# marksgraham/ddpm-ood

Hardware: AMD Instinct MI355X
Metric: reconstructions/sec (whole node), FashionMNIST 32x32 (higher is better)
Workload: dtype f32 (split-f16 MFMA products, fp32 accumulate)

## Files before the change

### ddpm_ood_amd/csrc/conv_wino44r.hip

```cpp
#include "wino44h_common.h"

namespace ddpm {

namespace {

constexpr int kVCB = 3 * kVSB;
static_assert(2 * kVCB == kRINGF * 4, "the V ring is the epilogue's four exchange slabs");

typedef int v4i_t __attribute__((ext_vector_type(4)));
typedef float v2f_t __attribute__((ext_vector_type(2)));

template <int O>
__device__ __forceinline__ void v_store_row_addtid(int m0base, const uint32_t (&hi6)[6], const uint32_t (&lo6)[6]) {
  asm volatile("s_mov_b32 m0, %0\n\ts_nop 1" ::"s"(m0base));
#pragma unroll
  for (int q = 0; q < 6; ++q) {
    asm volatile("ds_write_addtid_b32 %0 offset:%1" ::"v"(hi6[q]), "n"((2 * (O + q)) * (kT * 16)) : "memory");
    asm volatile("ds_write_addtid_b32 %0 offset:%1" ::"v"(lo6[q]), "n"((2 * (O + q) + 1) * (kT * 16)) : "memory");
  }
}

template <class T>
__device__ __forceinline__ const T *uniform_ptr(const T *p) {
  const uint64_t v = reinterpret_cast<uint64_t>(p);
  const uint32_t lo = __builtin_amdgcn_readfirstlane((uint32_t)v), hi = __builtin_amdgcn_readfirstlane((uint32_t)(v >> 32));
  return reinterpret_cast<const T *>(((uint64_t)hi << 32) | lo);
}

}

template <bool AFFINE, int NRT, int UIT, bool RES, bool D3 = false, bool UP = false>
__global__ __launch_bounds__(512, 2) void conv_wino44r_kernel(const ddpm_conv_desc a, const W44HGeom g) {
  extern __shared__ __attribute__((aligned(16))) float smem[];
  constexpr bool ONEIMG = UIT == 0;
  constexpr int NGS = ONEIMG ? 1 : NRT / UIT;
  constexpr int GD = ONEIMG ? NRT : UIT;
  float *const P = smem + kRINGF;

  const int tid = threadIdx.x;
  const int lane = tid & 63, wave = __builtin_amdgcn_readfirstlane(tid >> 6);
  const int l31 = lane & 31, lhi = lane >> 5;
  const int cb = wave & 1, pg = wave >> 1;
  const bool lateprod = wave < 4;
  const bool silu = a.act == DDPM_ACT_SILU;

  const int xcd = blockIdx.x & 7, wj = blockIdx.x >> 3;
  int kt = wj % g.KT, slot = (wj / g.KT) * 8 + xcd;
  if (g.xmap) {
    kt = xcd % g.KT;
    slot = wj * (8 / g.KT) + xcd / g.KT;
  }
  if (slot >= g.NS) return;
  const int split = slot % g.S;
  slot /= g.S;
  const int part = slot % g.parts, it0 = (slot / g.parts) * g.IPW;
  const int nitems = min(g.IPW, g.NIT - it0);
  const int r0 = part * g.TR;
  const int n_first = it0 * g.TI, n_end = n_first + nitems * g.TI;
  const int istep = g.rev ? -g.TI : g.TI;
  const int NCHs = g.NCH / g.S, ch_lo = split * NCHs;
  float *const outp = a.out + (size_t)split * g.pstride;

  f32x16 acc8;
  reserve_agprs();

  const __amdgpu_buffer_rsrc_t rs_u = __builtin_amdgcn_make_buffer_rsrc(
      const_cast<uint16_t *>(a.w_wino44h), 0, (int)((size_t)kX * a.Cout * g.Cin * g.nkd_w * 4), 0x00020000);
  const int ukt = ((kt * g.nkd_w + g.kd0) * g.NCHc + ch_lo) * 3;
  int ua = (3 * pg * 2 + lhi) * (kK * 16) + (cb * 32 + l31) * 16;
  int va = 3 * pg * (2 * kT * 16) + l31 * 16;

  auto barrier = [&]() __attribute__((always_inline)) {
    asm volatile("s_waitcnt lgkmcnt(0)\n\ts_barrier" ::: "memory");
    __builtin_amdgcn_sched_barrier(0);
  };
  auto zero_accumulators = [&]() __attribute__((always_inline)) {
    zero_pinned_tiles();
    float z;
    asm volatile("v_mov_b32 %0, 0" : "=v"(z));
    acc8 = f32x16{z, z, z, z, z, z, z, z, z, z, z, z, z, z, z, z};
  };

#ifdef W44R_PROBE
  if (blockIdx.x == 0 && lane == 0 && a.scratch) reinterpret_cast<unsigned long long *>(a.scratch)[512 + wave * 32 + 31] = __builtin_readcyclecounter();
#endif
  auto zero_borders = [&]() __attribute__((always_inline)) {
    const v4f z4 = {0.f, 0.f, 0.f, 0.f};
    for (int i = tid; i < g.HS; i += 512) *reinterpret_cast<v4f *>(P + 4 * i) = z4;
    __syncthreads();
  };

  using I0 = std::integral_constant<int, 0>;
  using I1 = std::integral_constant<int, 1>;
  using I2 = std::integral_constant<int, 2>;

#ifdef W44R_PROBE
  int probe_cc = -100;
  int n_idx_probe = 0;
#define W44R_STAMP(i)                                                                                                  \
  if (blockIdx.x == 0 && probe_cc >= 4 && probe_cc < 8 && lane == 0 && a.scratch)                                      \
    reinterpret_cast<unsigned long long *>(a.scratch)[((wave * 4 + (probe_cc - 4)) * 16 + (i)) & 511] = __builtin_readcyclecounter();
#define W44R_FSTAMP(i)                                                                                                 \
  if (blockIdx.x == 0 && n_idx_probe == 0 && lane == 0 && a.scratch)                                                    \
    reinterpret_cast<unsigned long long *>(a.scratch)[512 + wave * 32 + (i)] = __builtin_readcyclecounter();
#else
#define W44R_STAMP(i)
#define W44R_FSTAMP(i)
#endif
  W44R_FSTAMP(0)
  const int ptask = (wave & 3) == 3 ? -1 : wave - (wave >> 2);
  const int pst = (ptask & 1) * 16 + (lane >> 2), pj = lane & 3;
  int tb0;
  {
    const int per = g.TR * g.TWc;
    const int ti = pst / per, rem = pst - ti * per;
    const int tr = rem / g.TWc, tc = rem - tr * g.TWc;
    tb0 = (pj >> 1) * g.HS + 2 * (pj & 1) * g.PCH + ti * g.IS + 4 * tr * g.PW + 4 * tc;
  }
  int vw0 = pst * 16 + 4 * pj;
  auto produce = [&](auto tc_, int cc) __attribute__((always_inline)) {
    constexpr int t = decltype(tc_)::value;
    constexpr bool t0 = t == 0;
    constexpr float c1 = t0 ? -5.f : t == 1 ? -2.f : -0.5f, c2 = t0 ? 4.f : c1, bm = t0 ? 0.f : t == 1 ? 1.f : 2.f;
    asm volatile("" : "+v"(tb0), "+v"(vw0));
    const int pb0 = tb0 + (cc & 1) * 2 * g.HS;
    float cA[2][6], cB[2][6];
#pragma unroll
    for (int c = 0; c < 2; ++c) {
      const float *p = P + pb0 + c * g.PCH;
      float d4[6], d2[6], dx[6], dy[6], dz[6], dw[6];
      auto row = [&](int r, float (&dst)[6]) __attribute__((always_inline)) {
        const v4f lo = *reinterpret_cast<const v4f *>(p + r * g.PW);
        const v2f_t hi = *reinterpret_cast<const v2f_t *>(p + r * g.PW + 4);
        dst[0] = lo[0]; dst[1] = lo[1]; dst[2] = lo[2]; dst[3] = lo[3]; dst[4] = hi[0]; dst[5] = hi[1];
      };
      row(4, d4);
      row(2, d2);
      row(1, dw);
      row(t0 ? 5 : 3, dy);
      if (t0) {
        row(0, dx);
        row(3, dz);
      } else {
#pragma unroll
        for (int q = 0; q < 6; ++q) dx[q] = d2[q], dz[q] = dw[q];
      }
#pragma unroll
      for (int q = 0; q < 6; ++q) {
        const float wa = __builtin_fmaf(c2, dx[q], __builtin_fmaf(c1, d2[q], d4[q]));
        const float qq = __builtin_fmaf(c2, dw[q], __builtin_fmaf(c1, dz[q], dy[q]));
        cA[c][q] = __builtin_fmaf(bm, qq, wa);
        cB[c][q] = t0 ? qq : __builtin_fmaf(-bm, qq, wa);
      }
    }
    int vwa = vw0 + (cc & 1) * kVCB + t * kVSB;
    asm volatile("" : "+v"(vwa));
    float t0r[6], t1r[6];
    uint32_t hi6[6], lo6[6];
    bt6(cA[0], t0r);
    bt6(cA[1], t1r);
#pragma unroll
    for (int q = 0; q < 6; ++q) split_pair(t0r[q], t1r[q], hi6[q], lo6[q]);
    const int m0base = __builtin_amdgcn_readfirstlane((cc & 1) * kVCB + t * kVSB + (ptask & 1) * 256);
    v_store_row_addtid<0>(m0base, hi6, lo6);
    bt6(cB[0], t0r);
    bt6(cB[1], t1r);
#pragma unroll
    for (int q = 0; q < 6; ++q) split_pair(t0r[q], t1r[q], hi6[q], lo6[q]);
    v_store_row_addtid<6>(m0base, hi6, lo6);
  };
  auto produce_task = [&](int cc) __attribute__((always_inline)) {
    if (ptask < 0) return;
    const int t = ptask >> 1;
    if (t == 0) produce(I0{}, cc);
    else if (t == 1) produce(I1{}, cc);
    else produce(I2{}, cc);
  };

  const int sc = wave & 3, phalf = wave >> 2;
  const int row_lo = max(0, 4 * r0 - 1), row_hi = min(a.Ho, 4 * (r0 + g.TR) + 1);
  const int npx = (row_hi - row_lo) * a.Wo;
  const int dump = 4 * g.PCH + 1 + lane;
  int pix0, pw0, pixL = 0, pwL = 0;
  {
    const int e0 = lane;
    const bool valid = e0 < npx;
    auto src_of = [&](int row, int col) __attribute__((always_inline)) { return UP ? ((row >> 1) * (a.Wo >> 1) + (col >> 1)) * 4 : (row * a.Wo + col) * 4; };
    pix0 = valid ? src_of(row_lo + e0 / a.Wo, e0 % a.Wo) : (int)0x80000000;
    pw0 = valid ? sc * g.PCH + (row_lo + e0 / a.Wo - (4 * r0 - 1)) * g.PW + e0 % a.Wo + 1 : dump;
    if (ONEIMG) {
      const int eL = e0 + 64 * (NRT - 1);
      const bool vL = eL < npx;
      pixL = vL ? src_of(row_lo + eL / a.Wo, eL % a.Wo) : (int)0x80000000;
      pwL = vL ? sc * g.PCH + (row_lo + eL / a.Wo - (4 * r0 - 1)) * g.PW + eL % a.Wo + 1 : dump;
    }
  }
  const int prs = (64 / a.Wo) * g.PW;
  constexpr int kRoundBytes = UP ? 64 : 256;
  auto pix_of = [&](int k) __attribute__((always_inline)) { return ONEIMG ? (k == NRT - 1 ? pixL : pix0 + kRoundBytes * k) : pix0 + kRoundBytes * (k % GD); };
  auto pw_of = [&](int k) __attribute__((always_inline)) { return ONEIMG ? (k == NRT - 1 ? pwL : pw0 + k * prs) : pw0 + (k % GD) * prs + (k / GD) * g.IS; };
  const int bytes1 = a.B * a.C1 * (D3 ? g.CS : UP ? g.HWin : g.HW) * 4, bytes2 = a.B * a.C2 * g.HW * 4;
  const __amdgpu_buffer_rsrc_t rs_sc =
      __builtin_amdgcn_make_buffer_rsrc(const_cast<float *>(a.gscale), 0, AFFINE ? a.B * g.Cin * 4 : 0, 0x00020000);
  const __amdgpu_buffer_rsrc_t rs_sh =
      __builtin_amdgcn_make_buffer_rsrc(const_cast<float *>(a.gshift), 0, AFFINE ? a.B * g.Cin * 4 : 0, 0x00020000);
  int vzero;
  asm volatile("v_mov_b32 %0, 0" : "=v"(vzero));
  constexpr bool PACKED = UIT == 1;
  constexpr int NGL = PACKED ? 1 : NGS;
  float praw[2][NRT];
  float gs[2][NGL], gh[2][NGL];
  struct LoadCtx {
    __amdgpu_buffer_rsrc_t rs;
    int n_it, cx, cgl, cga, soff3;
    bool dok;
  };
  auto load_prep = [&](int cc, int n_cur, bool has_next) __attribute__((always_inline)) {
    LoadCtx L;
    const bool nxt = cc >= NCHs && has_next;
    const int cl = nxt ? cc - NCHs : min(max(cc, 0), NCHs - 1);
    L.n_it = nxt ? n_cur + istep : n_cur;
    int cg = (ch_lo + cl) * kC + phalf * 4 + sc;
    L.cga = cg;
    L.soff3 = 0;
    L.dok = true;
    if (D3) {
      const int kdi = cl / g.NCHc;
      cg = (cl - kdi * g.NCHc) * kC + phalf * 4 + sc;
      const int ni = min(L.n_it, g.NIMG - 1);
      const int nb = ni / g.D, dsl = ni - nb * g.D + g.kd0 + kdi - 1;
      L.dok = dsl >= 0 && dsl < g.D;
      L.soff3 = ((nb * a.C1 + cg) * g.D + (L.dok ? dsl : 0)) * g.HW * 4;
    }
    const bool first = cg < a.C1;
    L.rs = __builtin_amdgcn_make_buffer_rsrc(const_cast<float *>(first ? a.in1 : a.in2), 0, first ? bytes1 : bytes2, 0x00020000);
    L.cx = first ? a.C1 : a.C2;
    L.cgl = first ? cg : cg - a.C1;
    return L;
  };
  auto load_round = [&](const LoadCtx &L, auto setc, int k) __attribute__((always_inline)) {
    constexpr int S = decltype(setc)::value;
    const int ni = min(L.n_it + (ONEIMG ? 0 : k / GD), g.NIMG - 1);
    const int soff = D3 ? L.soff3 : (ni * L.cx + L.cgl) * (UP ? g.HWin : g.HW) * 4;
    const int voff = D3 && !L.dok ? (int)0x80000000 : pix_of(k);
    praw[S][k] = __builtin_bit_cast(float, __builtin_amdgcn_raw_buffer_load_b32(L.rs, voff, soff, 0));
  };
  auto load_affine = [&](const LoadCtx &L, auto setc, int i) __attribute__((always_inline)) {
    constexpr int S = decltype(setc)::value;
    if (AFFINE) {
      const int nb = min(L.n_it + i, g.NIMG - 1);
      const int goff = (nb * g.Cin + L.cga) * 4;
      const int voff = PACKED ? max(0, min(lane & 7, g.NIMG - 1 - L.n_it)) * (g.Cin * 4) : vzero;
      gs[S][i] = __builtin_bit_cast(float, __builtin_amdgcn_raw_buffer_load_b32(rs_sc, voff, goff, 0));
      gh[S][i] = __builtin_bit_cast(float, __builtin_amdgcn_raw_buffer_load_b32(rs_sh, voff, goff, 0));
    }
  };
  auto load_stage = [&](auto setc, int cc, int n_cur, bool has_next) __attribute__((always_inline)) {
    const LoadCtx L = load_prep(cc, n_cur, has_next);
#pragma unroll
    for (int k = 0; k < NRT; ++k) load_round(L, setc, k);
#pragma unroll
    for (int i = 0; i < NGL; ++i) load_affine(L, setc, i);
  };
  auto activate_round = [&](auto setc, int cc, int k) __attribute__((always_inline)) {
    constexpr int S = decltype(setc)::value;
    float *const Pr = P + (2 * (cc & 1) + phalf) * g.HS + pw_of(k);
    float sa = 0.f, sb = 0.f, ta = 0.f, tb = 0.f;
    if (AFFINE) {
      if (PACKED) {
        sa = __builtin_bit_cast(float, __builtin_amdgcn_readlane(__builtin_bit_cast(int, gs[S][0]), k / GD));
        sb = __builtin_bit_cast(float, __builtin_amdgcn_readlane(__builtin_bit_cast(int, gh[S][0]), k / GD));
      } else {
        sa = gs[S][k / GD];
        sb = gh[S][k / GD];
      }
      ta = -1.44269504088896341f * sa;
      tb = -1.44269504088896341f * sb;
    }
    auto act = [&](float x) __attribute__((always_inline)) {
      if (AFFINE) {
        const float v = __builtin_fmaf(x, sa, sb);
        const float t = __builtin_fmaf(x, ta, tb);
        return (kVScale * v) * __builtin_amdgcn_rcpf(1.0f + __builtin_amdgcn_exp2f(t));
      }
      return kVScaleRaw * (silu ? silu_fast(x) : x);
    };
    Pr[0] = act(praw[S][k]);
  };
  auto activate_stage = [&](auto setc, int cc) __attribute__((always_inline)) {
    asm volatile("" : "+v"(pix0), "+v"(pw0), "+v"(pixL), "+v"(pwL));
#pragma unroll
    for (int k = 0; k < NRT; ++k) activate_round(setc, cc, k);
  };

  constexpr int kAR = 6;
  h8 Ar[kAR];
  auto load_a = [&](int cl, int jj) __attribute__((always_inline)) {
    const int t = jj / 3, i = jj - 3 * t;
    const int c2 = min(cl, NCHs - 1);
    const v4i_t v = __builtin_bit_cast(v4i_t, __builtin_amdgcn_raw_buffer_load_b128(rs_u, ua + i * (2 * kK * 16), (ukt + 3 * c2 + t) * kUSB, 0));
    return __builtin_bit_cast(h8, v);
  };
  auto mfma_chunk = [&](auto parc, int cl, auto &&slice) __attribute__((always_inline)) {
    constexpr int PAR = decltype(parc)::value;
    asm volatile("" : "+v"(ua), "+v"(va));
    const int vb = va + (cl & 1) * kVCB;
    h8 Bh[2], Bl[2];
    Bh[0] = lds_b128(vb, 0);
    Bl[0] = lds_b128(vb, kT * 16);
#pragma unroll
    for (int jj = 0; jj < 9; ++jj) {
      if (jj < 8) {
        Bh[(jj + 1) & 1] = lds_b128(vb, ((jj + 1) / 3) * kVSB + 2 * ((jj + 1) % 3) * kT * 16);
        Bl[(jj + 1) & 1] = lds_b128(vb, ((jj + 1) / 3) * kVSB + (2 * ((jj + 1) % 3) + 1) * kT * 16);
        __builtin_amdgcn_sched_barrier(0);
      }
      const int ri = (PAR * 9 + jj) % kAR;
      if (jj == 8) {
        mfma_v_pair_wait0(acc8, Ar[ri], Bh[jj & 1], Bl[jj & 1]);
      } else {
        mfma_pin_wait<3>(jj, Ar[ri], Bh[jj & 1]);
        __builtin_amdgcn_sched_barrier(0);
        slice(jj, 0);
        __builtin_amdgcn_sched_barrier(0);
        asm volatile("s_waitcnt lgkmcnt(2)" ::: "memory");
        mfma_pin(jj, Ar[ri], Bl[jj & 1]);
      }
      __builtin_amdgcn_sched_barrier(0);
      Ar[ri] = load_a(jj + kAR < 9 ? cl : cl + 1, (jj + kAR) % 9);
      if (jj == 8) slice(jj, 0);
      slice(jj, 1);
      __builtin_amdgcn_sched_barrier(0);
    }
  };

  if (wave >= 4) asm volatile("s_setprio 1");
  for (int n_idx = 0; n_idx < nitems; ++n_idx) {
    const int n_cur = g.rev ? n_end - (n_idx + 1) * g.TI : n_first + n_idx * g.TI;
    const bool first_item = n_idx == 0 || !g.xitem;
    const bool has_next = g.xitem && n_idx + 1 < nitems;
#ifdef W44R_PROBE
    n_idx_probe = n_idx;
#endif
    W44R_FSTAMP(1)
    if (first_item) {
      load_stage(I0{}, 0, n_cur, has_next);
      load_stage(I1{}, 1, n_cur, has_next);
      if (n_idx == 0) zero_borders();
      W44R_FSTAMP(2)
      activate_stage(I0{}, 0);
      W44R_FSTAMP(3)
      load_stage(I0{}, 2, n_cur, has_next);
      activate_stage(I1{}, 1);
      W44R_FSTAMP(4)
      barrier();
    }
    W44R_FSTAMP(5)
#pragma unroll
    for (int jj = 0; jj < kAR; ++jj) Ar[jj] = load_a(0, jj);
    produce_task(0);
    zero_accumulators();
    W44R_FSTAMP(6)
    barrier();
    W44R_FSTAMP(7)
    const int pahead = lateprod ? 1 : 2;
    if (!lateprod) produce_task(1);
    auto interval = [&](auto parc, int cc) __attribute__((always_inline)) {
      constexpr int PAR = decltype(parc)::value;
      using SA = std::integral_constant<int, PAR>;
      using SL = std::integral_constant<int, 1 - PAR>;
#ifdef W44R_PROBE
      probe_cc = n_idx == 0 ? cc : -100;
#endif
      W44R_STAMP(0)
      const LoadCtx L = load_prep(cc + 3, n_cur, has_next);
      W44R_STAMP(1)
      asm volatile("" : "+v"(pix0), "+v"(pw0), "+v"(pixL), "+v"(pwL));
      mfma_chunk(parc, cc, [&](int jj, int part) __attribute__((always_inline)) {
        if ((jj & 1) == 0) {
          const int k = 2 * (jj / 2) + part;
          if (k < NRT) {
#pragma unroll
            for (int kk = 0; kk < NRT; ++kk)
              if (kk == k) activate_round(SA{}, cc + 2, kk);
          }
        } else {
#pragma unroll
          for (int k = 0; k < NRT; ++k)
            if (k / 3 == jj / 2 && (k % 3 == 0) == (part == 0)) load_round(L, SL{}, k);
          if (part == 1) {
#pragma unroll
            for (int i = 0; i < NGL; ++i)
              if (i == jj / 2) load_affine(L, SL{}, i);
          }
        }
      });
      W44R_STAMP(2)
      (void)activate_stage;
      W44R_STAMP(3)
      if (!lateprod) barrier();
      W44R_STAMP(4)
      if (cc + pahead < NCHs) produce_task(cc + pahead);
      W44R_STAMP(5)
      if (lateprod) barrier();
      W44R_STAMP(6)
    };
    for (int c = 0; c < NCHs; c += 2) {
      interval(I0{}, c);
      interval(I1{}, c + 1);
    }

    W44R_FSTAMP(8)
    asm volatile("s_nop 15\n\ts_nop 15\n\ts_nop 15\n\ts_nop 15" ::: "memory");
    int elane = lane;
    asm volatile("" : "+v"(elane));
    const int el31 = elane & 31, elhi = elane >> 5;
    const int per = g.TR * g.TWc;
    const int ti = el31 / per, rem = el31 - ti * per;
    const int tr = rem / g.TWc, tc = rem - tr * g.TWc;
    const int n = n_cur + ti, ncl = min(n, g.NIMG - 1);
    const int nbat = D3 ? ncl / g.D : ncl, dsl_o = D3 ? ncl - nbat * g.D : 0;
    const int cstr = D3 ? g.CS : g.HW;
    float *const XS = smem;
    float kOutScale, unused_umax;
    sload2(uniform_ptr(reinterpret_cast<const float *>(a.w_wino44h + (size_t)kX * a.Cout * g.Cin * 2 * g.nkd_w) + 1), kOutScale, unused_umax);
    (void)unused_umax;
    if (!AFFINE) kOutScale *= kVScale / kVScaleRaw;
    const int rsel = pg >> 1, cofs = 3 * (pg & 1);
    const int xb0 = (rsel ? 5 : 0) * 6 + cofs, xb1 = (rsel ? 2 : 1) * 6 + cofs, xb2 = (rsel ? 4 : 3) * 6 + cofs;
    float addv[4];
    if (ONEIMG) {
      const int co0 = kt * kK + cb * 32 + pg;
      float bs[8] = {0.f, 0.f, 0.f, 0.f, 0.f, 0.f, 0.f, 0.f}, ts[8] = {0.f, 0.f, 0.f, 0.f, 0.f, 0.f, 0.f, 0.f};
      const float *const tp = a.chan_add ? a.chan_add + (size_t)min(n_cur, g.NIMG - 1) * a.chan_add_stride + co0 : nullptr;
      if (a.bias && tp) sload8x2(uniform_ptr(a.bias + co0), uniform_ptr(tp), bs, ts);
      else if (a.bias) sload8(uniform_ptr(a.bias + co0), bs);
      else if (tp) sload8(uniform_ptr(tp), ts);
#pragma unroll
      for (int q = 0; q < 4; ++q) addv[q] = elhi ? bs[2 * q + 1] + ts[2 * q + 1] : bs[2 * q] + ts[2 * q];
    } else {
#pragma unroll
      for (int q = 0; q < 4; ++q) {
        const int co = kt * kK + cb * 32 + 8 * q + 4 * elhi + pg;
        addv[q] = (a.bias ? a.bias[co] : 0.f) + (a.chan_add ? a.chan_add[(size_t)ncl * a.chan_add_stride + co] : 0.f);
      }
    }
    const size_t co_e = (size_t)kt * kK + cb * 32 + 4 * elhi + pg;
    const size_t obase0 = (D3 ? (((size_t)nbat * a.Cout + co_e) * g.D + dsl_o) * g.HW : ((size_t)ncl * a.Cout + co_e) * g.HW) +
                          (size_t)(4 * (r0 + tr)) * a.Wo + 4 * tc;
    v4f res[4];
    auto load_res = [&](int q) __attribute__((always_inline)) {
#pragma unroll
      for (int k = 0; k < 4; ++k)
        res[k] = *reinterpret_cast<const v4f *>(a.residual + obase0 + (size_t)(8 * q) * cstr + (size_t)k * a.Wo);
    };
    if (RES) load_res(0);
    const bool emit_stats = !D3 && a.stats_out != nullptr && g.S == 1;
    auto pass = [&](auto qc) __attribute__((always_inline)) {
      constexpr int q = decltype(qc)::value;
      const size_t obase = obase0 + (size_t)(8 * q) * cstr;
      float st_p = 0.f, st_s1 = 0.f, st_s2 = 0.f;
#pragma unroll
      for (int hh = 0; hh < 2; ++hh) {
#pragma unroll
        for (int x3 = 0; x3 < 3; ++x3) {
          const int m0v = __builtin_amdgcn_readfirstlane(((x3 == 0 ? xb0 : x3 == 1 ? xb1 : xb2) * 128 + cb * 64 + hh * 2 * kXS) * 4);
          asm volatile("s_mov_b32 m0, %0\n\ts_nop 1" ::"s"(m0v));
#pragma unroll
          for (int xc = 0; xc < 3; ++xc) {
            const int x = 3 * x3 + xc;
#pragma unroll
            for (int r2 = 0; r2 < 2; ++r2) {
              const int rr = 2 * hh + r2;
              const float v = x == 8 ? acc8[4 * q + rr] : read_pinned(16 * (x & 7) + 4 * q + rr);
              if (r2 == 0) asm volatile("ds_write_addtid_b32 %0 offset:%1" ::"v"(v), "n"(xc * 512) : "memory");
              else asm volatile("ds_write_addtid_b32 %0 offset:%1" ::"v"(v), "n"(kXS * 4 + xc * 512) : "memory");
            }
          }
        }
      }
      asm volatile("s_waitcnt lgkmcnt(0)\n\ts_barrier" ::: "memory");
      const float *xr = XS + pg * kXS + cb * 64 + elane;
      const float ad = addv[q];
      auto half = [&](auto hc) __attribute__((always_inline)) {
        constexpr int h = decltype(hc)::value;
        float w[2][6];
#pragma unroll
        for (int jj = 0; jj < 6; ++jj) {
          const float m1 = xr[(1 * 6 + jj) * 128], m2 = xr[(2 * 6 + jj) * 128], m3 = xr[(3 * 6 + jj) * 128],
                      m4 = xr[(4 * 6 + jj) * 128];
          if (h == 0) {
            const float m0 = xr[(0 * 6 + jj) * 128];
            w[0][jj] = (m0 + (m1 + m2)) + (m3 + m4);
            w[1][jj] = __builtin_fmaf(2.f, m3 - m4, m1 - m2);
          } else {
            const float m5 = xr[(5 * 6 + jj) * 128];
            w[0][jj] = __builtin_fmaf(4.f, m3 + m4, m1 + m2);
            w[1][jj] = __builtin_fmaf(8.f, m3 - m4, m1 - m2) + m5;
          }
        }
#pragma unroll
        for (int kk = 0; kk < 2; ++kk) {
          const int k = 2 * h + kk;
          float y[4];
          at4(w[kk][0], w[kk][1], w[kk][2], w[kk][3], w[kk][4], w[kk][5], y);
          v4f o = v4f{__builtin_fmaf(y[0], kOutScale, ad), __builtin_fmaf(y[1], kOutScale, ad),
                      __builtin_fmaf(y[2], kOutScale, ad), __builtin_fmaf(y[3], kOutScale, ad)};
          if (RES) o += res[k];
          if (D3 && a.out_act == DDPM_ACT_RELU) o = v4f{fmaxf(o[0], 0.f), fmaxf(o[1], 0.f), fmaxf(o[2], 0.f), fmaxf(o[3], 0.f)};
          if (n < g.NIMG) *reinterpret_cast<v4f *>(outp + obase + (size_t)k * a.Wo) = o;
          if (emit_stats) {
            if (k == 0) st_p = o[0];
            const v4f dd = o - st_p;
            st_s1 += (dd[0] + dd[1]) + (dd[2] + dd[3]);
            st_s2 += (dd[0] * dd[0] + dd[1] * dd[1]) + (dd[2] * dd[2] + dd[3] * dd[3]);
          }
        }
      };
      half(I0{});
      v4f r01[2];
      if (RES && q < 3) {
#pragma unroll
        for (int k = 0; k < 2; ++k)
          r01[k] = *reinterpret_cast<const v4f *>(a.residual + obase + (size_t)8 * cstr + (size_t)k * a.Wo);
      }
      half(I1{});
      if (RES && q < 3) {
        res[0] = r01[0];
        res[1] = r01[1];
#pragma unroll
        for (int k = 2; k < 4; ++k)
          res[k] = *reinterpret_cast<const v4f *>(a.residual + obase + (size_t)8 * cstr + (size_t)k * a.Wo);
      }
      if (emit_stats) {
        float mean = st_p + st_s1 * (1.f / 16.f);
        float m2 = fmaxf(st_s2 - st_s1 * st_s1 * (1.f / 16.f), 0.f);
        group_moments_last_lane(mean, m2, 16.f, per);
        if (rem == per - 1 && n < g.NIMG) {
          const size_t co = (size_t)kt * kK + cb * 32 + 8 * q + 4 * elhi + pg;
          *reinterpret_cast<float2 *>(a.stats_out + (((size_t)n * a.Cout + co) * g.parts + part) * 2) = make_float2(mean, m2);
        }
      }
      asm volatile("s_waitcnt lgkmcnt(0)\n\ts_barrier" ::: "memory");
    };
    W44R_FSTAMP(9)
    pass(I0{});
    W44R_FSTAMP(10)
    pass(I1{});
    W44R_FSTAMP(11)
    pass(I2{});
    W44R_FSTAMP(12)
    pass(std::integral_constant<int, 3>{});
    W44R_FSTAMP(13)
    __builtin_amdgcn_sched_barrier(0);
  }
}

void w44r_relayout(const ddpm_conv_desc &d, W44HGeom &g) {
  const int w = d.Wo + 2;
  int pw = (w + 3) & ~3;
  if (g.TWc == 8) while (pw % 16 != 8) pw += 4;
  if (g.TWc == 4) while (pw % 16 != 4) pw += 4;
  g.PW = pw;
  g.IS = g.prow * g.PW;
  if (g.TI == 8) while (g.IS % 16 != 8) g.IS += 4;
  g.PCH = g.TI * g.IS;
  while (g.PCH % 32 != 16) g.PCH += 1;
  g.HS = 4 * g.PCH + 272;
}

int launch_conv_wino44r(const ddpm_conv_desc &dk, const W44HGeom &g, size_t lds, hipStream_t s) {
  typedef void (*kern_t)(const ddpm_conv_desc, const W44HGeom);
#define W44R_K(A, N, U) {conv_wino44r_kernel<A, N, U, false>, conv_wino44r_kernel<A, N, U, true>}
  static const kern_t kerns[2][4][2] = {
      {W44R_K(false, 9, 0), W44R_K(false, 10, 0), W44R_K(false, 8, 4), W44R_K(false, 8, 1)},
      {W44R_K(true, 9, 0), W44R_K(true, 10, 0), W44R_K(true, 8, 4), W44R_K(true, 8, 1)}};
#undef W44R_K
  static bool attr_done = false;
  if (!attr_done) {
    for (int i = 0; i < 16; ++i)
      (void)hipFuncSetAttribute(reinterpret_cast<const void *>(kerns[i / 8][i / 2 % 4][i % 2]),
                                hipFuncAttributeMaxDynamicSharedMemorySize, 160 * 1024);
    attr_done = true;
  }
  const int shape = g.TI == 1 ? (g.NRT == 9 ? 0 : 1) : g.UI == 4 ? 2 : 3;
  kern_t kern = kerns[dk.gscale ? 1 : 0][shape][dk.residual ? 1 : 0];
  if (g.up) {
    static const kern_t kerns_up[4] = {conv_wino44r_kernel<false, 9, 0, false, false, true>, conv_wino44r_kernel<false, 10, 0, false, false, true>,
                                       conv_wino44r_kernel<false, 8, 4, false, false, true>, conv_wino44r_kernel<false, 8, 1, false, false, true>};
    static bool attr_up_done = false;
    if (!attr_up_done) {
      for (int i = 0; i < 4; ++i)
        (void)hipFuncSetAttribute(reinterpret_cast<const void *>(kerns_up[i]), hipFuncAttributeMaxDynamicSharedMemorySize, 160 * 1024);
      attr_up_done = true;
    }
    kern = kerns_up[shape];
  }
  if (dk.dims == 3) {
    static const kern_t kerns3d[2][2] = {{conv_wino44r_kernel<false, 9, 0, false, true>, conv_wino44r_kernel<false, 9, 0, true, true>},
                                         {conv_wino44r_kernel<false, 10, 0, false, true>, conv_wino44r_kernel<false, 10, 0, true, true>}};
    static bool attr3_done = false;
    if (!attr3_done) {
      for (int i = 0; i < 4; ++i)
        (void)hipFuncSetAttribute(reinterpret_cast<const void *>(kerns3d[i / 2][i % 2]), hipFuncAttributeMaxDynamicSharedMemorySize,
                                  160 * 1024);
      attr3_done = true;
    }
    kern = kerns3d[g.NRT == 9 ? 0 : 1][dk.residual ? 1 : 0];
  }
  hipLaunchKernelGGL(kern, dim3(g.grid), dim3(512), lds, s, dk, g);
  DDPM_CHECK_LAUNCH();
  return 0;
}

}
```

Before: 1072.

## Skip structurally zero Winograd positions in nearest-upsample conv path

For the UP (nearest-neighbour upsampled input) variant, the Winograd F(4x4,3x3) input transform is specialised: duplicated input pixels make some of the 36 transform positions zero. Each wave group now handles only the 25 non-zero positions (6 or 7 per pg, with a per-lane job table) and drops the rest. The change adds a dedicated produce/MFMA/epilogue path and shrinks MFMA and LDS traffic on that path, at the cost of more code, an extra A register, uneven work (pg0 does 7 jobs), and exactness depending on the zero pattern holding.

```diff
diff --git a/ddpm_ood_amd/csrc/conv_wino44r.hip b/ddpm_ood_amd/csrc/conv_wino44r.hip
--- a/ddpm_ood_amd/csrc/conv_wino44r.hip
+++ b/ddpm_ood_amd/csrc/conv_wino44r.hip
@@ -18,6 +18,21 @@
     asm volatile("ds_write_addtid_b32 %0 offset:%1" ::"v"(hi6[q]), "n"((2 * (O + q)) * (kT * 16)) : "memory");
     asm volatile("ds_write_addtid_b32 %0 offset:%1" ::"v"(lo6[q]), "n"((2 * (O + q) + 1) * (kT * 16)) : "memory");
   }
+}
+
+constexpr int w44r_up_job(int idx) {
+  const int t = idx < 10 ? 0 : idx < 15 ? 1 : 2;
+  const int k = idx - (t == 0 ? 0 : t == 1 ? 10 : 15);
+  const int s = k < 2 ? k : k < 7 ? k + 1 : k + 2;
+  const int row = t == 0 ? (s < 6 ? 0 : 5) : t == 1 ? 1 : (s < 6 ? 3 : 4);
+  return (t * kVSB + 2 * s * (kT * 16)) | ((row * 6 + s % 6) << 16);
+}
+static_assert(kUSB == 2 * kVSB && 3 * kVSB < 65536, "w44r_up_job: U offset = 2 x V offset, below bit 16");
+
+template <int T, int S>
+__device__ __forceinline__ void v_store_pos_addtid(uint32_t hi, uint32_t lo) {
+  asm volatile("ds_write_addtid_b32 %0 offset:%1" ::"v"(hi), "n"(T * kVSB + (2 * S) * (kT * 16)) : "memory");
+  asm volatile("ds_write_addtid_b32 %0 offset:%1" ::"v"(lo), "n"(T * kVSB + (2 * S + 1) * (kT * 16)) : "memory");
 }
 
 template <class T>
@@ -69,6 +84,16 @@
   const int ukt = ((kt * g.nkd_w + g.kd0) * g.NCHc + ch_lo) * 3;
   int ua = (3 * pg * 2 + lhi) * (kK * 16) + (cb * 32 + l31) * 16;
   int va = 3 * pg * (2 * kT * 16) + l31 * 16;
+  int upj[7] = {0, 0, 0, 0, 0, 0, 0};
+  bool up7 = false;
+  if constexpr (UP) {
+#pragma unroll
+    for (int j = 0; j < 7; ++j)
+      upj[j] = __builtin_amdgcn_readfirstlane(pg == 0 ? w44r_up_job(j) : pg == 1 ? w44r_up_job(7 + j) : pg == 2 ? w44r_up_job(13 + j) : w44r_up_job(19 + (j < 6 ? j : 5)));
+    up7 = pg == 0;
+    ua = lhi * (kK * 16) + (cb * 32 + l31) * 16;
+    va = l31 * 16;
+  }
 
   auto barrier = [&]() __attribute__((always_inline)) {
     asm volatile("s_waitcnt lgkmcnt(0)\n\ts_barrier" ::: "memory");
@@ -76,6 +101,7 @@
   };
   auto zero_accumulators = [&]() __attribute__((always_inline)) {
     zero_pinned_tiles();
+    if constexpr (UP) return;
     float z;
     asm volatile("v_mov_b32 %0, 0" : "=v"(z));
     acc8 = f32x16{z, z, z, z, z, z, z, z, z, z, z, z, z, z, z, z};
@@ -169,9 +195,93 @@
     for (int q = 0; q < 6; ++q) split_pair(t0r[q], t1r[q], hi6[q], lo6[q]);
     v_store_row_addtid<6>(m0base, hi6, lo6);
   };
+  auto produce_up = [&](auto kc_, int cc) __attribute__((always_inline)) {
+    constexpr int K = decltype(kc_)::value;
+    asm volatile("" : "+v"(tb0));
+    const int pb0 = tb0 + (cc & 1) * 2 * g.HS;
+    float X[2][4], Y[2][4], Z[2][4];
+#pragma unroll
+    for (int c = 0; c < 2; ++c) {
+      const float *p = P + pb0 + c * g.PCH;
+      float rb[4], rc[4], re[4];
+      auto row = [&](int r, float (&dst)[4]) __attribute__((always_inline)) {
+        const v4f lo = *reinterpret_cast<const v4f *>(p + r * g.PW);
+        const v2f_t hi = *reinterpret_cast<const v2f_t *>(p + r * g.PW + 4);
+        dst[0] = lo[0]; dst[1] = lo[2]; dst[2] = hi[0]; dst[3] = hi[1];
+      };
+      row(2, rb);
+      row(4, rc);
+      if (K == 0) row(0, re);
+      if (K == 1) row(5, re);
+#pragma unroll
+      for (int q = 0; q < 4; ++q) {
+        const float w12 = __builtin_fmaf(-2.f, rb[q], __builtin_fmaf(-2.f, rb[q], rc[q]));
+        const float w34 = __builtin_fmaf(-0.5f, rb[q], __builtin_fmaf(-0.5f, rb[q], rc[q]));
+        if constexpr (K == 0) {
+          X[c][q] = __builtin_fmaf(4.f, re[q], __builtin_fmaf(-5.f, rb[q], rc[q]));
+          Y[c][q] = __builtin_fmaf(1.f, w12, w12);
+        } else if constexpr (K == 1) {
+          X[c][q] = __builtin_fmaf(4.f, rb[q], __builtin_fmaf(-5.f, rc[q], re[q]));
+          Y[c][q] = __builtin_fmaf(-2.f, w34, w34);
+        } else {
+          X[c][q] = __builtin_fmaf(2.f, w34, w34);
+          Y[c][q] = __builtin_fmaf(-2.f, w34, w34);
+          Z[c][q] = __builtin_fmaf(1.f, w12, w12);
+        }
+      }
+    }
+    auto rp = [&](const float (&x)[4], float (&o)[5]) __attribute__((always_inline)) {
+      const float pp = __builtin_fmaf(-4.f, x[1], x[2]), rr = x[2] - x[1];
+      o[0] = __builtin_fmaf(4.f, x[0], __builtin_fmaf(-5.f, x[1], x[2]));
+      o[1] = pp + pp;
+      o[2] = __builtin_fmaf(2.f, rr, rr);
+      o[3] = __builtin_fmaf(-2.f, rr, rr);
+      o[4] = __builtin_fmaf(4.f, x[1], __builtin_fmaf(-5.f, x[2], x[3]));
+    };
+    auto st = [&](auto tc_, auto sc_, float v0, float v1) __attribute__((always_inline)) {
+      uint32_t h, l;
+      split_pair(v0, v1, h, l);
+      v_store_pos_addtid<decltype(tc_)::value, decltype(sc_)::value>(h, l);
+    };
+    using std::integral_constant;
+    const int m0base = __builtin_amdgcn_readfirstlane((cc & 1) * kVCB + (ptask & 1) * 256);
+    float a0[5], a1[5];
+    rp(X[0], a0);
+    rp(X[1], a1);
+    asm volatile("s_mov_b32 m0, %0\n\ts_nop 1" ::"s"(m0base));
+    constexpr int TX = K == 0 ? 0 : K == 1 ? 0 : 2, SX = K == 1 ? 6 : 0;
+    st(integral_constant<int, TX>{}, integral_constant<int, SX + 0>{}, a0[0], a1[0]);
+    st(integral_constant<int, TX>{}, integral_constant<int, SX + 1>{}, a0[1], a1[1]);
+    st(integral_constant<int, TX>{}, integral_constant<int, SX + 3>{}, a0[2], a1[2]);
+    st(integral_constant<int, TX>{}, integral_constant<int, SX + 4>{}, a0[3], a1[3]);
+    st(integral_constant<int, TX>{}, integral_constant<int, SX + 5>{}, a0[4], a1[4]);
+    rp(Y[0], a0);
+    rp(Y[1], a1);
+    asm volatile("s_mov_b32 m0, %0\n\ts_nop 1" ::"s"(m0base));
+    if constexpr (K == 2) {
+      st(I2{}, integral_constant<int, 10>{}, a0[3], a1[3]);
+      st(I2{}, integral_constant<int, 11>{}, a0[4], a1[4]);
+      rp(Z[0], a0);
+      rp(Z[1], a1);
+      asm volatile("s_mov_b32 m0, %0\n\ts_nop 1" ::"s"(m0base));
+      st(I1{}, integral_constant<int, 4>{}, a0[3], a1[3]);
+      st(I1{}, integral_constant<int, 5>{}, a0[4], a1[4]);
+    } else {
+      constexpr int TY = K == 0 ? 1 : 2, SY = K == 0 ? 0 : 6;
+      st(integral_constant<int, TY>{}, integral_constant<int, SY + 0>{}, a0[0], a1[0]);
+      st(integral_constant<int, TY>{}, integral_constant<int, SY + 1>{}, a0[1], a1[1]);
+      st(integral_constant<int, TY>{}, integral_constant<int, SY + 3>{}, a0[2], a1[2]);
+    }
+  };
   auto produce_task = [&](int cc) __attribute__((always_inline)) {
     if (ptask < 0) return;
     const int t = ptask >> 1;
+    if constexpr (UP) {
+      if (t == 0) produce_up(I0{}, cc);
+      else if (t == 1) produce_up(I1{}, cc);
+      else produce_up(I2{}, cc);
+      return;
+    }
     if (t == 0) produce(I0{}, cc);
     else if (t == 1) produce(I1{}, cc);
     else produce(I2{}, cc);
@@ -294,7 +404,7 @@
   };
 
   constexpr int kAR = 6;
-  h8 Ar[kAR];
+  h8 Ar[UP ? 7 : kAR];
   auto load_a = [&](int cl, int jj) __attribute__((always_inline)) {
     const int t = jj / 3, i = jj - 3 * t;
     const int c2 = min(cl, NCHs - 1);
@@ -331,6 +441,53 @@
       if (jj == 8) slice(jj, 0);
       slice(jj, 1);
       __builtin_amdgcn_sched_barrier(0);
+    }
+  };
+
+  auto load_a_up = [&](int cl, int job) __attribute__((always_inline)) {
+    const int c2 = min(cl, NCHs - 1);
+    const v4i_t v = __builtin_bit_cast(v4i_t, __builtin_amdgcn_raw_buffer_load_b128(rs_u, ua, (ukt + 3 * c2) * kUSB + 2 * (job & 0xffff), 0));
+    return __builtin_bit_cast(h8, v);
+  };
+  auto mfma_chunk_up = [&](int cl, auto &&slice) __attribute__((always_inline)) {
+    asm volatile("" : "+v"(ua), "+v"(va));
+    const int vb = va + (cl & 1) * kVCB;
+    h8 Bh[2], Bl[2];
+    auto read_b = [&](int slot, int job) __attribute__((always_inline)) {
+      const int ad = vb + (job & 0xffff);
+      Bh[slot] = lds_b128(ad, 0);
+      Bl[slot] = lds_b128(ad, kT * 16);
+    };
+    auto job = [&](auto jc, auto lastc) __attribute__((always_inline)) {
+      constexpr int j = decltype(jc)::value;
+      constexpr bool last = decltype(lastc)::value;
+      if constexpr (!last) {
+        read_b((j + 1) & 1, upj[j + 1]);
+        __builtin_amdgcn_sched_barrier(0);
+      }
+      mfma_pin_wait<last ? 1 : 3>(j, Ar[j], Bh[j & 1]);
+      __builtin_amdgcn_sched_barrier(0);
+      slice(j, 0);
+      __builtin_amdgcn_sched_barrier(0);
+      if constexpr (last) asm volatile("s_waitcnt lgkmcnt(0)" ::: "memory");
+      else asm volatile("s_waitcnt lgkmcnt(2)" ::: "memory");
+      mfma_pin(j, Ar[j], Bl[j & 1]);
+      __builtin_amdgcn_sched_barrier(0);
+      Ar[j] = load_a_up(cl + 1, upj[j]);
+      slice(j, 1);
+      __builtin_amdgcn_sched_barrier(0);
+    };
+    read_b(0, upj[0]);
+    job(I0{}, std::false_type{});
+    job(I1{}, std::false_type{});
+    job(I2{}, std::false_type{});
+    job(std::integral_constant<int, 3>{}, std::false_type{});
+    job(std::integral_constant<int, 4>{}, std::false_type{});
+    if (up7) {
+      job(std::integral_constant<int, 5>{}, std::false_type{});
+      job(std::integral_constant<int, 6>{}, std::true_type{});
+    } else {
+      job(std::integral_constant<int, 5>{}, std::true_type{});
     }
   };
 
@@ -356,8 +513,14 @@
       barrier();
     }
     W44R_FSTAMP(5)
-#pragma unroll
-    for (int jj = 0; jj < kAR; ++jj) Ar[jj] = load_a(0, jj);
+    if constexpr (UP) {
+#pragma unroll
+      for (int jj = 0; jj < 6; ++jj) Ar[jj] = load_a_up(0, upj[jj]);
+      if (up7) Ar[6] = load_a_up(0, upj[6]);
+    } else {
+#pragma unroll
+      for (int jj = 0; jj < kAR; ++jj) Ar[jj] = load_a(0, jj);
+    }
     produce_task(0);
     zero_accumulators();
     W44R_FSTAMP(6)
@@ -376,6 +539,20 @@
       const LoadCtx L = load_prep(cc + 3, n_cur, has_next);
       W44R_STAMP(1)
       asm volatile("" : "+v"(pix0), "+v"(pw0), "+v"(pixL), "+v"(pwL));
+      if constexpr (UP) {
+        mfma_chunk_up(cc, [&](int jj, int part) __attribute__((always_inline)) {
+          if (jj >= 6) return;
+          const int k = 2 * jj + part;
+#pragma unroll
+          for (int kk = 0; kk < NRT; ++kk)
+            if (kk == k) activate_round(SA{}, cc + 2, kk);
+          if (part == 1) {
+#pragma unroll
+            for (int kk = 0; kk < NRT; ++kk)
+              if (kk / 2 == jj) load_round(L, SL{}, kk);
+          }
+        });
+      } else
       mfma_chunk(parc, cc, [&](int jj, int part) __attribute__((always_inline)) {
         if ((jj & 1) == 0) {
           const int k = 2 * (jj / 2) + part;
@@ -460,6 +637,19 @@
       constexpr int q = decltype(qc)::value;
       const size_t obase = obase0 + (size_t)(8 * q) * cstr;
       float st_p = 0.f, st_s1 = 0.f, st_s2 = 0.f;
+      if constexpr (UP) {
+#pragma unroll
+        for (int hh = 0; hh < 2; ++hh) {
+#pragma unroll
+          for (int j = 0; j < 7; ++j) {
+            if (j == 6 && !up7) continue;
+            const int m0v = __builtin_amdgcn_readfirstlane(((upj[j] >> 16) * 128 + cb * 64 + hh * 2 * kXS) * 4);
+            asm volatile("s_mov_b32 m0, %0\n\ts_nop 1" ::"s"(m0v));
+            asm volatile("ds_write_addtid_b32 %0 offset:%1" ::"v"(read_pinned(16 * j + 4 * q + 2 * hh)), "n"(0) : "memory");
+            asm volatile("ds_write_addtid_b32 %0 offset:%1" ::"v"(read_pinned(16 * j + 4 * q + 2 * hh + 1)), "n"(kXS * 4) : "memory");
+          }
+        }
+      } else
 #pragma unroll
       for (int hh = 0; hh < 2; ++hh) {
 #pragma unroll
@@ -487,7 +677,12 @@
         float w[2][6];
 #pragma unroll
         for (int jj = 0; jj < 6; ++jj) {
-          const float m1 = xr[(1 * 6 + jj) * 128], m2 = xr[(2 * 6 + jj) * 128], m3 = xr[(3 * 6 + jj) * 128],
+          if (UP && jj == 2) {
+            w[0][jj] = 0.f;
+            w[1][jj] = 0.f;
+            continue;
+          }
+          const float m1 = xr[(1 * 6 + jj) * 128], m2 = UP ? 0.f : xr[(2 * 6 + jj) * 128], m3 = xr[(3 * 6 + jj) * 128],
                       m4 = xr[(4 * 6 + jj) * 128];
           if (h == 0) {
             const float m0 = xr[(0 * 6 + jj) * 128];
```

After: 1090, median of 6. +1.7%, better.
